# rohitsinghlab/SAME

Measured on AMD Instinct MI355X. Metric: cell-pairs/sec on 100k×100k cost build + edge-cross sweep; % HBM roofline, higher is better.
Workload: dtype f64

## Files before the change

### same_amd/csrc/common.h

```cpp
#pragma once
#include <hip/hip_runtime.h>

#include <cstdint>
#include <cstdio>
#include <cstring>
#include <string>
#include <vector>

#include "same_hip_diag.h"

struct ncclComm;

enum Slot {
    SL_A = 0, SL_R, SL_AXY, SL_RXY, SL_PAIRS, SL_OUT0, SL_OUT1, SL_OUT2, SL_TRIS, SL_MATCH,
    SL_SIGN, SL_SIZE, SL_TYPE, SL_FLAG0, SL_FLAG1, SL_FLAG2, SL_COUNTS, SL_X, SL_MASK,
    SL_K_HIST, SL_K_RANK, SL_K_SXY, SL_K_SIDX, SL_K_BBOX, SL_K_START,
    SL_Q_START, SL_Q_RANK, SL_Q_SXY, SL_Q_SIDX,
    SL_COUNT
};

struct same_spread_alloc {
    char *va = nullptr;
    size_t bytes = 0;
    std::vector<void *> handles;
// ... 102 lines not shown
}
template <typename T>
inline int up_as(same_ctx *ctx, Slot s, const T *host, size_t n, T **out) {
    void *p = nullptr;
    int rc = same_up(ctx, s, host, n * sizeof(T), &p);
    *out = static_cast<T *>(p);
    return rc;
}

static inline int64_t ceil_div(int64_t a, int64_t b) { return (a + b - 1) / b; }

int check_index_range(same_ctx *ctx, const int32_t *idx, int64_t n, int64_t lo, int64_t hi, const char *what);

struct same_pair_csr {
    std::vector<int32_t> prow, order, where, csr;
    std::vector<double> ccsr;
};
inline int same_pairs_by_row(same_ctx *ctx, const int32_t *pairs, const double *costs, int64_t P, int64_t n_m, int64_t n_r, same_pair_csr *out) {
    std::vector<int32_t> &prow = out->prow, &order = out->order, &where = out->where, &csr = out->csr;
    prow.assign((size_t)n_m + 1, 0);
    order.resize((size_t)P);
    where.resize((size_t)P);
    csr.resize((size_t)P * 2);
    out->ccsr.resize((size_t)P);
    for (int64_t p = 0; p < P; ++p) {
        const int32_t i = pairs[2 * p], j = pairs[2 * p + 1];
        REQUIRE(ctx, i >= 0 && i < n_m && j >= 0 && j < n_r);
        ++prow[(size_t)i + 1];
    }
    for (int64_t i = 0; i < n_m; ++i) prow[(size_t)i + 1] += prow[(size_t)i];
    {
        std::vector<int32_t> at(prow.begin(), prow.end() - 1);
        for (int64_t p = 0; p < P; ++p) {
            const int32_t q = at[(size_t)pairs[2 * p]]++;
            order[(size_t)q] = (int32_t)p;
            where[(size_t)p] = q;
        }
    }
    std::vector<int64_t> seen((size_t)n_r, -1);
    for (int64_t i = 0; i < n_m; ++i)
        for (int32_t q = prow[(size_t)i]; q < prow[(size_t)i + 1]; ++q) {
            const int32_t p = order[(size_t)q], j = pairs[2 * (int64_t)p + 1];
            if (seen[(size_t)j] == i) {
                ctx->err = "invalid argument: a (row, column) pair given twice";
                return SAME_EINVAL;
            }
            seen[(size_t)j] = i;
            csr[2 * (size_t)q] = (int32_t)i;
            csr[2 * (size_t)q + 1] = j;
            out->ccsr[(size_t)q] = costs[p];
        }
    return SAME_OK;
}

int same_pair_rowmin_core(same_ctx *ctx, const int32_t *dpairs, const double *dcosts, int64_t P, int64_t n_m, double *dout);
int same_greedy_core(same_ctx *ctx, const int32_t *dpairs, const double *dcosts, int64_t P, int64_t n_m, int64_t n_r,
                     const uint8_t *dprefer, int32_t *dmatch_pair, int *out_rounds);

constexpr int SAME_GREEDY_BATCH_MAX = 64;
struct same_greedy_state {
    uint8_t *alive = nullptr;
    uint8_t *used = nullptr;
    unsigned long long *key[2] = {nullptr, nullptr};
    unsigned *idx[2] = {nullptr, nullptr};
    unsigned long long *sel = nullptr;
    bool float_costs = false;
};
int same_greedy_rounds_core(same_ctx *ctx, const int32_t *dpairs, const double *dcosts, int64_t P, const unsigned long long *dP,
                            int64_t n_m, int64_t n_r, const same_greedy_state &st, int32_t *dmatch_pair, int first, int count);

constexpr int SAME_LAUNCH_WINDOWS = 8;
struct same_greedy_job {
    const int32_t *pairs = nullptr;
    const double *costs = nullptr;
    int64_t P = 0, n_m = 0, n_r = 0;
    same_greedy_state st;
    int32_t *match_pair = nullptr;
};
int same_greedy_rounds_batch_core(same_ctx *ctx, const same_greedy_job *jobs, int n_jobs, int first, int count);

int same_sort_u64_core(same_ctx *ctx, unsigned long long *dkey, int64_t n_pad);
int same_merge_dedup_core(same_ctx *ctx, const uint8_t *dviol, unsigned viol_mask, const int32_t *dwin, const int32_t *da, const int32_t *dr,
                          int64_t n, int32_t *dout, unsigned long long *dtotal);

struct same_knn_index;
struct same_knn_window_job {
    const int32_t *rows_m = nullptr;
    const unsigned long long *dn_m = nullptr;
    int64_t cap_m = 0;
    const int32_t *rows_r = nullptr;
    const unsigned long long *dn_r = nullptr;
    double box[4] = {0, 0, 0, 0};
    int32_t *idx = nullptr, *cnt = nullptr;
};
int same_knn_window_batch_core(same_ctx *ctx, const same_knn_index *ix, const double *dmov_xy, const same_knn_window_job *jobs, int n_jobs, int k);
struct same_cost_window_job {
    const int32_t *rows = nullptr;
    const unsigned long long *dn = nullptr;
    int64_t cap = 0;
    const int32_t *idx = nullptr;
    void *out = nullptr;
};
int same_padded_cost_window_batch_core(same_ctx *ctx, int cost_f32, const void *dA, const void *dR, int T, const void *daxy_c, const void *drxy_c,
                                       const same_cost_window_job *jobs, int n_jobs, int k, double w);
```

### same_amd/csrc/merge.hip

```cpp
#include <algorithm>

#include "common.h"
#include "scan.h"

namespace {

constexpr int SORT_BLOCK = 2048;

__global__ __launch_bounds__(256) void merge_key_kernel(const uint8_t *__restrict__ viol, unsigned viol_mask, const int32_t *__restrict__ window, int64_t n,
                                                          int64_t n_pad, unsigned long long *__restrict__ key) {
    const int64_t i = (int64_t)blockIdx.x * blockDim.x + threadIdx.x;
    if (i >= n_pad) return;
    key[i] = i < n ? ((unsigned long long)((viol[i] & viol_mask) ? 1 : 0) << 63) | ((unsigned long long)(uint32_t)window[i] << 32) | (unsigned long long)i
                   : ~0ull;
}

__global__ __launch_bounds__(256) void bitonic_global_kernel(unsigned long long *__restrict__ key, int64_t n_pad, int64_t j, int64_t k) {
    const int64_t t = (int64_t)blockIdx.x * blockDim.x + threadIdx.x;
    if (t >= n_pad / 2) return;
    const int64_t lo = ((t / j) * 2 * j) + (t % j), hi = lo + j;
    const bool up = (lo & k) == 0;
    const unsigned long long a = key[lo], b = key[hi];
    if ((a > b) == up) { key[lo] = b; key[hi] = a; }
}

__global__ __launch_bounds__(1024) void bitonic_lds_kernel(unsigned long long *__restrict__ key, int64_t k, int j_top) {
    __shared__ unsigned long long s[SORT_BLOCK];
    const int64_t base = (int64_t)blockIdx.x * SORT_BLOCK;
    s[threadIdx.x] = key[base + threadIdx.x];
    s[threadIdx.x + 1024] = key[base + threadIdx.x + 1024];
    __syncthreads();
    for (int j = j_top; j >= 1; j >>= 1) {
        const int t = threadIdx.x;
        const int lo = ((t / j) * 2 * j) + (t % j), hi = lo + j;
        const bool up = ((base + lo) & k) == 0;
        const unsigned long long a = s[lo], b = s[hi];
        if ((a > b) == up) { s[lo] = b; s[hi] = a; }
        __syncthreads();
    }
    key[base + threadIdx.x] = s[threadIdx.x];
    key[base + threadIdx.x + 1024] = s[threadIdx.x + 1024];
}

__global__ __launch_bounds__(1024) void bitonic_lds_head_kernel(unsigned long long *__restrict__ key) {
    __shared__ unsigned long long s[SORT_BLOCK];
    const int64_t base = (int64_t)blockIdx.x * SORT_BLOCK;
    s[threadIdx.x] = key[base + threadIdx.x];
    s[threadIdx.x + 1024] = key[base + threadIdx.x + 1024];
    __syncthreads();
    for (int k = 2; k <= SORT_BLOCK; k <<= 1)
        for (int j = k >> 1; j >= 1; j >>= 1) {
            const int t = threadIdx.x;
            const int lo = ((t / j) * 2 * j) + (t % j), hi = lo + j;
            const bool up = ((base + lo) & k) == 0;
            const unsigned long long a = s[lo], b = s[hi];
            if ((a > b) == up) { s[lo] = b; s[hi] = a; }
            __syncthreads();
        }
    key[base + threadIdx.x] = s[threadIdx.x];
    key[base + threadIdx.x + 1024] = s[threadIdx.x + 1024];
}

__device__ __forceinline__ uint64_t mix64(uint64_t x) {
    x ^= x >> 30; x *= 0xbf58476d1ce4e5b9ull;
    x ^= x >> 27; x *= 0x94d049bb133111ebull;
    return x ^ (x >> 31);
}

constexpr unsigned long long EMPTY = ~0ull;

__device__ __forceinline__ int64_t pair_slot(unsigned long long *__restrict__ tkey, int64_t mask, unsigned long long pair) {
    int64_t h = (int64_t)(mix64(pair) & (uint64_t)mask);
    for (;;) {
        const unsigned long long seen = atomicCAS(&tkey[h], EMPTY, pair);
        if (seen == EMPTY || seen == pair) return h;
        h = (h + 1) & mask;
    }
}

__global__ __launch_bounds__(256) void merge_first_kernel(const unsigned long long *__restrict__ key, int64_t n, const int32_t *__restrict__ a_code,
                                                            const int32_t *__restrict__ r_code, unsigned long long *__restrict__ tkey,
                                                            unsigned int *__restrict__ tfirst, int64_t mask) {
    const int64_t s = (int64_t)blockIdx.x * blockDim.x + threadIdx.x;
    if (s >= n) return;
    const uint32_t row = (uint32_t)key[s];
    const unsigned long long pair = ((unsigned long long)(uint32_t)a_code[row] << 32) | (uint32_t)r_code[row];
    atomicMin(&tfirst[pair_slot(tkey, mask, pair)], (unsigned int)s);
}

__global__ __launch_bounds__(scan::NT) void merge_compact_kernel(const unsigned long long *__restrict__ key, int64_t n, const int32_t *__restrict__ a_code,
                                                                  const int32_t *__restrict__ r_code, unsigned long long *__restrict__ tkey,
                                                                  const unsigned int *__restrict__ tfirst, int64_t mask,
                                                                  unsigned long long *__restrict__ status, int32_t *__restrict__ out_rows,
                                                                  unsigned long long *__restrict__ out_total) {
    __shared__ scan::Shared sh;
    auto keep_of = [&](int64_t q) -> bool {
        if (q >= n) return false;
        const uint32_t row = (uint32_t)key[q];
        const unsigned long long pair = ((unsigned long long)(uint32_t)a_code[row] << 32) | (uint32_t)r_code[row];
        return tfirst[pair_slot(tkey, mask, pair)] == (unsigned int)q;
    };
    const int64_t s0 = (int64_t)blockIdx.x * scan::NT + threadIdx.x;
    const bool keep = keep_of(s0);
    auto val = [&](int64_t q) { return scan::Pair{(q == s0 ? keep : keep_of(q)) ? 1u : 0u, 0u}; };
    scan::Pair through;
    const scan::Pair off = scan::exclusive(status, (int)blockIdx.x, val, sh, &through);
    if (keep) out_rows[off.a] = (int32_t)(uint32_t)key[s0];
    if (blockIdx.x == gridDim.x - 1 && threadIdx.x == 0) *out_total = through.a;
}

}

int same_sort_u64_core(same_ctx *ctx, unsigned long long *dkey, int64_t n_pad) {
    REQUIRE(ctx, n_pad >= SORT_BLOCK && (n_pad & (n_pad - 1)) == 0);
    hipLaunchKernelGGL(bitonic_lds_head_kernel, dim3((unsigned)(n_pad / SORT_BLOCK)), dim3(1024), 0, ctx->stream, dkey);
    for (int64_t k = 2 * SORT_BLOCK; k <= n_pad; k <<= 1) {
        for (int64_t j = k >> 1; j >= SORT_BLOCK; j >>= 1)
            hipLaunchKernelGGL(bitonic_global_kernel, dim3((unsigned)ceil_div(n_pad / 2, 256)), dim3(256), 0, ctx->stream, dkey, n_pad, j, k);
        hipLaunchKernelGGL(bitonic_lds_kernel, dim3((unsigned)(n_pad / SORT_BLOCK)), dim3(1024), 0, ctx->stream, dkey, k, SORT_BLOCK / 2);
    }
    HIP_TRY(ctx, hipGetLastError());
    return SAME_OK;
}

int same_merge_dedup_core(same_ctx *ctx, const uint8_t *dviol, unsigned viol_mask, const int32_t *dwin, const int32_t *da, const int32_t *dr,
                          int64_t n, int32_t *dout, unsigned long long *dtotal) {
    REQUIRE(ctx, n > 0 && n < ((int64_t)1 << 30));
    int64_t n_pad = SORT_BLOCK;
    while (n_pad < n) n_pad <<= 1;
    int64_t slots = 2;
    while (slots < 2 * n) slots <<= 1;
    unsigned long long *dkey, *dtkey, *dstatus;
    unsigned int *dtfirst;
    const size_t st_words = scan::status_bytes(n) / 8;
    SAME_TRY(slot_as(ctx, SL_X, (size_t)n_pad, &dkey));
    SAME_TRY(slot_as(ctx, SL_OUT0, (size_t)slots, &dtkey));
    SAME_TRY(slot_as(ctx, SL_OUT1, (size_t)slots, &dtfirst));
    SAME_TRY(slot_as(ctx, SL_MASK, st_words, &dstatus));
    SAME_FILL(ctx, dtkey, 0xFF, (size_t)slots * 8);
    SAME_FILL(ctx, dtfirst, 0xFF, (size_t)slots * 4);
    SAME_FILL(ctx, dstatus, 0, st_words * 8);
    SAME_LAUNCH(ctx, merge_key_kernel, dim3((unsigned)ceil_div(n_pad, 256)), dim3(256), 0, dviol, viol_mask, dwin, n, n_pad, dkey);
    SAME_TRY(same_sort_u64_core(ctx, dkey, n_pad));
    const unsigned grid = (unsigned)ceil_div(n, 256);
    SAME_LAUNCH(ctx, merge_first_kernel, dim3(grid), dim3(256), 0, dkey, n, da, dr, dtkey, dtfirst, slots - 1);
    SAME_LAUNCH(ctx, merge_compact_kernel, dim3(scan::blocks_for(n)), dim3(scan::NT), 0, dkey, n, da, dr, dtkey, dtfirst, slots - 1,
                scan::arg(dstatus), dout, dtotal);
    HIP_TRY(ctx, hipGetLastError());
    return SAME_OK;
}

extern "C" int same_merge_dedup(same_ctx *ctx, const uint8_t *viol, const int32_t *window_id, const int32_t *aligned_code,
                                const int32_t *ref_code, int64_t n, int32_t *out_rows, int64_t *out_n) {
    REQUIRE(ctx, ctx && out_n && n >= 0 && n < ((int64_t)1 << 30));
    *out_n = 0;
    if (n == 0) return SAME_OK;
    REQUIRE(ctx, viol && window_id && aligned_code && ref_code && out_rows);
    for (int64_t i = 0; i < n; ++i)
        if (window_id[i] < 0 || aligned_code[i] < 0 || ref_code[i] < 0) {
            ctx->err = "same_merge_dedup: window ids and id codes must be non-negative";
            return SAME_ERANGE;
        }
    SAME_TRY(same_use(ctx));
    uint8_t *dviol;
    int32_t *dwin, *da, *dr, *dout;
    unsigned long long *dtotal;
    SAME_TRY(up_as(ctx, SL_FLAG0, viol, (size_t)n, &dviol));
    SAME_TRY(up_as(ctx, SL_PAIRS, window_id, (size_t)n, &dwin));
    SAME_TRY(up_as(ctx, SL_MATCH, aligned_code, (size_t)n, &da));
    SAME_TRY(up_as(ctx, SL_TRIS, ref_code, (size_t)n, &dr));
    SAME_TRY(slot_as(ctx, SL_OUT2, (size_t)n + 4, &dout));
    dtotal = reinterpret_cast<unsigned long long *>(dout + (((size_t)n + 1) & ~size_t(1)));
    SAME_TRY(same_merge_dedup_core(ctx, dviol, 0xFFu, dwin, da, dr, n, dout, dtotal));
    unsigned long long total = 0;
    SAME_TRY(same_down(ctx, &total, dtotal, sizeof total));
    HIP_TRY(ctx, hipStreamSynchronize(ctx->stream));
    REQUIRE(ctx, (int64_t)total <= n);
    SAME_TRY(same_down(ctx, out_rows, dout, (size_t)total * sizeof(int32_t)));
    HIP_TRY(ctx, hipStreamSynchronize(ctx->stream));
    *out_n = (int64_t)total;
    return SAME_OK;
}
```

### same_amd/csrc/window_merge.hip

```cpp
#include "window_internal.h"


namespace {

using namespace devmath;
using namespace win;
using scan::Pair;

struct CollectArgs {
    const int32_t *match_row;
    const uint8_t *pflag;
    const int32_t *rows_ua;
    const double *axy;
    int64_t n;
    double tx0, tx1, ty0, ty1;
    int32_t wid, pos;
};

__device__ __forceinline__ bool central(const CollectArgs &w, int64_t c) {
    if (c >= w.n || w.match_row[c] < 0) return false;
    const double2_t p = ld2(w.axy, c);
    return p.x >= w.tx0 && p.x < w.tx1 && p.y >= w.ty0 && p.y < w.ty1;
}

// ... 23 lines not shown
                                                                  int64_t cap) {
    __shared__ scan::Shared sh;
    const CollectArgs &w = b.w[blockIdx.y];
    if ((int64_t)blockIdx.x * scan::NT >= w.n) return;
    auto val = [&](int64_t c) { return Pair{central(w, c) ? 1u : 0u, 0u}; };
    Pair through;
    const Pair off = scan::exclusive(status + blockIdx.y * status_stride, (int)blockIdx.x, val, sh, &through);
    const int64_t c = (int64_t)blockIdx.x * scan::NT + threadIdx.x;
    if (!central(w, c)) return;
    unsigned long long at = dcount[0] + off.a;
    for (unsigned q = 0; q < blockIdx.y; ++q) at += dcount[2 + q];
    if ((int64_t)at >= cap) return;
    acc.a_row[at] = w.rows_ua[c];
    acc.r_row[at] = w.match_row[c];
    acc.flags[at] = w.pflag[c];
    acc.wid[at] = w.wid;
    acc.pos[at] = w.pos;
    acc.cidx[at] = (int32_t)c;
}

__global__ void collect_bump_kernel(unsigned long long *dcount, int n_w) {
    unsigned long long add = 0;
    for (int q = 0; q < n_w; ++q) {
        add += dcount[2 + q];
        dcount[2 + q] = 0ull;
    }
    dcount[0] += add;
}

__global__ __launch_bounds__(256) void codes_kernel(const int32_t *__restrict__ a_row, const int32_t *__restrict__ r_row, int64_t n,
                                                     const int32_t *__restrict__ a_codes, const int32_t *__restrict__ r_codes,
                                                     int32_t *__restrict__ ac, int32_t *__restrict__ rc) {
    const int64_t i = (int64_t)blockIdx.x * blockDim.x + threadIdx.x;
    if (i >= n) return;
    ac[i] = a_codes ? a_codes[a_row[i]] : a_row[i];
    rc[i] = r_codes ? r_codes[r_row[i]] : r_row[i];
}

__global__ __launch_bounds__(256) void degree_kernel(const int32_t *__restrict__ kept, const unsigned long long *__restrict__ dm, int64_t bound,
                                                      const int32_t *__restrict__ ac, const int32_t *__restrict__ rc,
                                                      unsigned *__restrict__ deg_a, unsigned *__restrict__ deg_r) {
    const int64_t i = (int64_t)blockIdx.x * blockDim.x + threadIdx.x;
    if (i >= bound || i >= (int64_t)*dm) return;
    const int32_t row = kept[i];
    atomicAdd(&deg_a[ac[row]], 1u);
    atomicAdd(&deg_r[rc[row]], 1u);
}

struct SeamArgs {
    const int32_t *near_start;
    const double *near_boxes;
    const double *mov_xy, *ref_xy;
    int n_pos, all_seam;
    double reach;
};

__device__ __forceinline__ bool seam_of(const SeamArgs &s, int32_t pos, int32_t a_row, int32_t r_row) {
    if (s.all_seam) return true;
    if (!s.near_start) return false;
    if (pos < 0 || pos >= s.n_pos) return true;
    const int32_t b = s.near_start[pos], e = s.near_start[pos + 1];
    if (b == e) return false;
    const double2_t a = ld2(s.mov_xy, a_row), r = ld2(s.ref_xy, r_row);
    for (int32_t q = b; q < e; ++q) {
        const double x0 = s.near_boxes[4 * (int64_t)q], x1 = s.near_boxes[4 * (int64_t)q + 1], y0 = s.near_boxes[4 * (int64_t)q + 2],
                     y1 = s.near_boxes[4 * (int64_t)q + 3];
        if (a.x >= x0 && a.x < x1 && a.y >= y0 && a.y < y1) return true;
        if (r.x >= x0 - s.reach && r.x <= x1 + s.reach && r.y >= y0 - s.reach && r.y <= y1 + s.reach) return true;
    }
    return false;
}

__global__ __launch_bounds__(256) void classify_kernel(const int32_t *__restrict__ kept, const unsigned long long *__restrict__ dm, int64_t bound,
                                                        const int32_t *__restrict__ ac, const int32_t *__restrict__ rc,
                                                        const unsigned *__restrict__ deg_a, const unsigned *__restrict__ deg_r,
                                                        const int32_t *__restrict__ a_row, const int32_t *__restrict__ r_row,
                                                        const int32_t *__restrict__ pos, SeamArgs seams, uint8_t *__restrict__ cls,
                                                        int32_t *__restrict__ row_of) {
    const int64_t i = (int64_t)blockIdx.x * blockDim.x + threadIdx.x;
    if (i >= bound || i >= (int64_t)*dm) return;
    const int32_t row = kept[i];
    const bool lone = deg_a[ac[row]] == 1u && deg_r[rc[row]] == 1u;
    const bool seam = seam_of(seams, pos[row], a_row[row], r_row[row]);
    cls[i] = seam ? 3 : (lone ? 0 : 1);
    if (lone && !seam) row_of[ac[row]] = row;
}

__global__ __launch_bounds__(scan::NT) void rest_kernel(const int32_t *__restrict__ kept, const unsigned long long *__restrict__ dm,
                                                         const uint8_t *__restrict__ cls, const int32_t *__restrict__ ac,
                                                         const int32_t *__restrict__ rc, AccRows acc, unsigned long long *__restrict__ status,
                                                         RestRec *__restrict__ out, unsigned long long *__restrict__ out_total) {
    __shared__ scan::Shared sh;
    const int64_t m = (int64_t)*dm;
    auto val = [&](int64_t i) { return Pair{i < m && cls[i] != 0 ? 1u : 0u, 0u}; };
    Pair through;
    const Pair off = scan::exclusive(status, (int)blockIdx.x, val, sh, &through);
    const int64_t i = (int64_t)blockIdx.x * scan::NT + threadIdx.x;
    if (i < m && cls[i] != 0) {
        const int32_t row = kept[i];
        out[off.a] = RestRec{row, ac[row], rc[row], acc.wid[row], acc.pos[row], acc.cidx[row], (acc.flags[row] & 3u) | (cls[i] == 3 ? 4u : 0u)};
    }
    if (blockIdx.x == gridDim.x - 1 && threadIdx.x == 0) *out_total = through.a;
}

__global__ __launch_bounds__(256) void winners_kernel(const int32_t *__restrict__ rows, int64_t n, const int32_t *__restrict__ ac,
                                                       int32_t *__restrict__ row_of) {
    const int64_t i = (int64_t)blockIdx.x * blockDim.x + threadIdx.x;
    if (i < n) row_of[ac[rows[i]]] = rows[i];
}

__global__ __launch_bounds__(scan::NT) void final_kernel(const int32_t *__restrict__ row_of, int64_t n_codes, AccRows acc,
                                                          unsigned long long *__restrict__ status, FinalRec *__restrict__ out,
                                                          unsigned long long *__restrict__ out_total) {
    __shared__ scan::Shared sh;
    auto val = [&](int64_t c) { return Pair{c < n_codes && row_of[c] >= 0 ? 1u : 0u, 0u}; };
    Pair through;
    const Pair off = scan::exclusive(status, (int)blockIdx.x, val, sh, &through);
    const int64_t c = (int64_t)blockIdx.x * scan::NT + threadIdx.x;
    if (c < n_codes && row_of[c] >= 0) {
        const int32_t row = row_of[c];
        out[off.a] = FinalRec{acc.a_row[row], acc.r_row[row], acc.cidx[row], acc.wid[row], acc.pos[row], acc.flags[row] & 3u};
    }
    if (blockIdx.x == gridDim.x - 1 && threadIdx.x == 0) *out_total = through.a;
}

constexpr int MAX_EXTRA_COLUMNS = 4;
struct ExtraColumns {
    const unsigned long long *mov[MAX_EXTRA_COLUMNS], *ref[MAX_EXTRA_COLUMNS];
    int n_mov, n_ref;
};
__global__ __launch_bounds__(256) void table_columns_kernel(const FinalRec *__restrict__ rows, int64_t n, const double *__restrict__ mov_types, int T,
                                                            const double *__restrict__ mov_xy, const double *__restrict__ ref_xy, ExtraColumns ex,
                                                            unsigned long long *__restrict__ out) {
    const int64_t i = (int64_t)blockIdx.x * blockDim.x + threadIdx.x;
    if (i >= n) return;
    const FinalRec rec = rows[i];
    const int64_t a = rec.a_row, r = rec.r_row;
    const unsigned long long *__restrict__ t = reinterpret_cast<const unsigned long long *>(mov_types) + a * T;
    int64_t col = 0;
    for (int q = 0; q < T; ++q) out[(col++) * n + i] = t[q];
    const unsigned long long *pa = reinterpret_cast<const unsigned long long *>(mov_xy) + 2 * a,
                             *pr = reinterpret_cast<const unsigned long long *>(ref_xy) + 2 * r;
    out[(col++) * n + i] = pa[0];
    out[(col++) * n + i] = pa[1];
    out[(col++) * n + i] = pr[0];
    out[(col++) * n + i] = pr[1];
    for (int q = 0; q < ex.n_mov; ++q) out[(col++) * n + i] = ex.mov[q][a];
    for (int q = 0; q < ex.n_ref; ++q) out[(col++) * n + i] = ex.ref[q][r];
    out[(col++) * n + i] = (unsigned long long)(long long)rec.cidx;
    out[(col++) * n + i] = (unsigned long long)(long long)rec.wid;
    out[(col++) * n + i] = (unsigned long long)(long long)rec.pos;
    uint8_t *bytes = reinterpret_cast<uint8_t *>(out + col * n);
    bytes[i] = (uint8_t)((rec.flags >> 1) & 1u);
    bytes[n + i] = (uint8_t)(rec.flags & 1u);
}

AccRows rows_of(const same_merge_acc *a) { return AccRows{a->a_row, a->r_row, a->wid, a->pos, a->cidx, a->flags}; }

void free_rows(same_merge_acc *a) {
    for (void *p : {(void *)a->a_row, (void *)a->r_row, (void *)a->wid, (void *)a->pos, (void *)a->cidx, (void *)a->flags})
        if (p) (void)hipFree(p);
    a->a_row = a->r_row = a->wid = a->pos = a->cidx = nullptr;
    a->flags = nullptr;
    a->cap = 0;
}

int reserve_rows(same_merge_acc *a, int64_t need, int64_t have) {
    if (need <= a->cap) return SAME_OK;
    same_ctx *ctx = a->ctx;
    HIP_TRY(ctx, hipStreamSynchronize(ctx->stream));
    const int64_t cap = std::max<int64_t>(need + need / 4, 4096);
    int32_t **fields[5] = {&a->a_row, &a->r_row, &a->wid, &a->pos, &a->cidx};
    int32_t *olds[5], *news[5] = {nullptr, nullptr, nullptr, nullptr, nullptr};
    uint8_t *old_flags = a->flags, *new_flags = nullptr;
    for (int q = 0; q < 5; ++q) olds[q] = *fields[q];
    hipError_t e = hipSuccess;
    for (int q = 0; q < 5 && e == hipSuccess; ++q) {
        e = hipMalloc(reinterpret_cast<void **>(&news[q]), (size_t)cap * sizeof(int32_t));
        if (e == hipSuccess && have) e = hipMemcpyAsync(news[q], olds[q], (size_t)have * sizeof(int32_t), hipMemcpyDeviceToDevice, ctx->stream);
    }
    if (e == hipSuccess) e = hipMalloc(reinterpret_cast<void **>(&new_flags), (size_t)cap);
    if (e == hipSuccess && have) e = hipMemcpyAsync(new_flags, old_flags, (size_t)have, hipMemcpyDeviceToDevice, ctx->stream);
    if (e == hipSuccess) e = hipStreamSynchronize(ctx->stream);
    if (e != hipSuccess) {
        for (int q = 0; q < 5; ++q)
// ... 145 lines not shown
    a->loaded_codes_a = n_codes_a;
    a->loaded_codes_r = n_codes_r;
    const unsigned long long cnt[2] = {(unsigned long long)n, 0ull};
    SAME_COPY(ctx, a->dcount, cnt, sizeof cnt, hipMemcpyHostToDevice);
    if (n) {
        int32_t *const dst[5] = {a->a_row, a->r_row, a->wid, a->pos, a->cidx};
        const int32_t *const src[5] = {a_code, r_code, window_ids, pos, cidx};
        for (int f = 0; f < 5; ++f) SAME_COPY(ctx, dst[f], src[f], (size_t)n * sizeof(int32_t), hipMemcpyHostToDevice);
        SAME_COPY(ctx, a->flags, flags, (size_t)n, hipMemcpyHostToDevice);
    }
    SAME_WAIT(ctx);
    return SAME_OK;
}

int same_window_collect(same_window *const *windows, int n_windows, same_merge_acc *a, const double *trims, const int32_t *window_ids,
                        const int32_t *plan_pos) {
    same_ctx *ctx = nullptr;
    SAME_TRY(check_batch(windows, n_windows, &ctx));
    REQUIRE(ctx, a && a->ctx == ctx && trims && window_ids && plan_pos && !a->resolved);
    int64_t add = 0;
    for (int i = 0; i < n_windows; ++i) {
        REQUIRE(ctx, windows[i]->has_results() && window_ids[i] >= 0);
        add += windows[i]->cur.n_ua;
    }
    REQUIRE(ctx, a->bound + add < ((int64_t)1 << 30));
    SAME_TRY(same_use(ctx));
    if (a->bound + add > a->cap) {
        unsigned long long have = 0;
        HIP_TRY(ctx, hipMemcpyAsync(&have, a->dcount, sizeof have, hipMemcpyDeviceToHost, ctx->stream));
        HIP_TRY(ctx, hipStreamSynchronize(ctx->stream));
        SAME_TRY(reserve_rows(a, a->bound + add, (int64_t)have));
    }
    a->bound += add;
    int64_t most = 0;
    for (int i = 0; i < n_windows; ++i) most = std::max(most, windows[i]->cur.n_ua);
    const int64_t stride = (int64_t)(scan::status_bytes(most) / 8);
    SAME_TRY(ensure(ctx, a->scan_words, (size_t)stride * 8 * SAME_LAUNCH_WINDOWS));
    unsigned long long *words = static_cast<unsigned long long *>(a->scan_words.p);
    for (int g = 0; g < n_windows; g += SAME_LAUNCH_WINDOWS) {
        Batch<CollectArgs> b{};
        int n_g = 0;
        int64_t most_g = 0;
        for (int i = g; i < n_windows && i < g + SAME_LAUNCH_WINDOWS; ++i) {
            const same_window *w = windows[i];
            if (w->cur.n_ua == 0) continue;
            const double *t = trims + 4 * i;
            b.w[n_g++] = CollectArgs{w->match_row, w->pflag, w->cur.rows_ua, w->cur.axy_c, w->cur.n_ua, t[0], t[1], t[2], t[3], window_ids[i], plan_pos[i]};
            most_g = std::max(most_g, w->cur.n_ua);
        }
        if (!n_g) continue;
        const dim3 grid(scan::blocks_for(most_g), (unsigned)n_g);
        SAME_LAUNCH(ctx, collect_count_kernel, grid, dim3(scan::NT), 0, b, a->dcount + 2, words, stride);
        SAME_LAUNCH(ctx, collect_write_kernel, grid, dim3(scan::NT), 0, b, a->dcount, scan::arg(words), stride, rows_of(a), a->cap);
        SAME_LAUNCH(ctx, collect_bump_kernel, dim3(1), dim3(1), 0, a->dcount, n_g);
    }
    HIP_TRY(ctx, hipGetLastError());
    return SAME_OK;
}

int same_merge_acc_resolve(same_merge_acc *const *accs, int n_accs, const same_section *mov, const same_section *ref, int64_t *out_counts) {
    if (!accs || n_accs < 1 || !accs[0]) return SAME_EINVAL;
    same_merge_acc *a = accs[0];
    same_ctx *ctx = a->ctx;
    REQUIRE(ctx, n_accs <= 64 && out_counts);
    const bool loaded = a->loaded != 0;
    REQUIRE(ctx, loaded ? n_accs == 1 : (mov && ref && mov->ctx->device == ctx->device && ref->ctx->device == ctx->device));
    for (int q = 0; q < n_accs; ++q) {
        REQUIRE(ctx, accs[q] && accs[q]->ctx->device == ctx->device && !accs[q]->resolved);
        for (int p = 0; p < q; ++p) REQUIRE(ctx, accs[p] != accs[q]);
    }
    for (int q = 0; q < 4; ++q) out_counts[q] = 0;
    SAME_TRY(same_use(ctx));
    int64_t n = 0;
    SAME_TRY(lay_end_to_end(accs, n_accs, &n));
    for (int q = 0; q < n_accs; ++q) accs[q]->resolved = 1;
    a->n_rows = n;
    a->n_codes_a = loaded ? a->loaded_codes_a : (mov->id_codes ? mov->n_codes : mov->n);
    const int64_t n_codes_a = std::max<int64_t>(a->n_codes_a, 1),
                  n_codes_r = std::max<int64_t>(loaded ? a->loaded_codes_r : (ref->id_codes ? ref->n_codes : ref->n), 1);
    const int32_t *codes_a = loaded ? nullptr : mov->id_codes, *codes_r = loaded ? nullptr : ref->id_codes;
    const int64_t nn = std::max<int64_t>(n, 1);
    unsigned long long *status, *counters;
    unsigned *deg_a, *deg_r;
    int32_t *kept;
    uint8_t *cls;
    size_t zero_bytes = 0;
    auto lay = [&](Carver cv) {
        status = cv.scan_words(nn);
        counters = cv.take<unsigned long long>(8);
        deg_a = cv.take<unsigned>((size_t)n_codes_a);
        deg_r = cv.take<unsigned>((size_t)n_codes_r);
        zero_bytes = cv.off;
        a->row_of = cv.take<int32_t>((size_t)n_codes_a);
        a->ac = cv.take<int32_t>((size_t)nn);
        a->rc = cv.take<int32_t>((size_t)nn);
        kept = cv.take<int32_t>((size_t)nn);
        cls = cv.take<uint8_t>((size_t)nn);
        return cv.off;
    };
    SAME_TRY(ensure(ctx, a->work, lay(Carver())));
    lay(Carver(a->work.p));
    SAME_FILL(ctx, a->work.p, 0, zero_bytes);
    SAME_FILL(ctx, a->row_of, 0xFF, (size_t)n_codes_a * 4);
    a->counters = counters;
    SAME_TRY(ensure(ctx, a->out, (size_t)nn * sizeof(RestRec)));
    RestRec *rest = static_cast<RestRec *>(a->out.p);
    if (n) {
        SAME_LAUNCH(ctx, codes_kernel, dim3(grid_for(n)), dim3(256), 0, a->a_row, a->r_row, n, codes_a, codes_r, a->ac, a->rc);
        SAME_TRY(same_merge_dedup_core(ctx, a->flags, 1u, a->wid, a->ac, a->rc, n, kept, counters));
        SAME_LAUNCH(ctx, degree_kernel, dim3(grid_for(n)), dim3(256), 0, kept, counters, n, a->ac, a->rc, deg_a, deg_r);
        const SeamArgs seams{a->n_pos ? static_cast<const int32_t *>(a->near_start.p) : nullptr, static_cast<const double *>(a->near_boxes.p),
                             loaded ? nullptr : mov->xy, loaded ? nullptr : ref->xy, a->n_pos, a->all_seam, a->reach};
        SAME_LAUNCH(ctx, classify_kernel, dim3(grid_for(n)), dim3(256), 0, kept, counters, n, a->ac, a->rc, deg_a, deg_r, a->a_row, a->r_row, a->pos,
                    seams, cls, a->row_of);
        SAME_LAUNCH(ctx, rest_kernel, dim3(scan::blocks_for(n)), dim3(scan::NT), 0, kept, counters, cls, a->ac, a->rc, rows_of(a), scan::arg(status), rest,
                    counters + 1);
        HIP_TRY(ctx, hipGetLastError());
        unsigned long long hc[2] = {0, 0};
        SAME_COPY(ctx, hc, counters, sizeof hc, hipMemcpyDeviceToHost);
        SAME_WAIT(ctx);
        REQUIRE(ctx, (int64_t)hc[0] <= n && (int64_t)hc[1] <= (int64_t)hc[0]);
        a->n_kept = (int64_t)hc[0];
        a->n_rest = (int64_t)hc[1];
    }
    a->host.resize((size_t)a->n_rest * sizeof(RestRec) + 64);
    if (a->n_rest) {
        SAME_COPY(ctx, a->host.data(), rest, (size_t)a->n_rest * sizeof(RestRec), hipMemcpyDeviceToHost);
        SAME_WAIT(ctx);
    }
    out_counts[0] = a->n_rows;
    out_counts[1] = a->n_kept;
    out_counts[2] = a->n_rest;
    out_counts[3] = a->n_kept - a->n_rest;
    return SAME_OK;
}

int same_merge_acc_plain(same_merge_acc *const *accs, int n_accs, int64_t *out_n_rows) {
    if (!accs || n_accs < 1 || !accs[0]) return SAME_EINVAL;
    same_merge_acc *a = accs[0];
    same_ctx *ctx = a->ctx;
    REQUIRE(ctx, n_accs <= 64 && out_n_rows && !a->loaded);
    for (int q = 0; q < n_accs; ++q) {
        REQUIRE(ctx, accs[q] && accs[q]->ctx->device == ctx->device && !accs[q]->resolved);
        for (int p = 0; p < q; ++p) REQUIRE(ctx, accs[p] != accs[q]);
    }
    *out_n_rows = 0;
    SAME_TRY(same_use(ctx));
    int64_t n = 0;
    SAME_TRY(lay_end_to_end(accs, n_accs, &n));
    for (int q = 0; q < n_accs; ++q) accs[q]->resolved = 2;
    a->n_rows = a->n_kept = a->n_final = n;
    a->n_rest = 0;
    a->final_on_host = 0;
    a->merged = 0;
    SAME_TRY(ensure(ctx, a->out, (size_t)std::max<int64_t>(n, 1) * sizeof(FinalRec)));
    if (n) SAME_LAUNCH(ctx, plain_kernel, dim3(grid_for(n)), dim3(256), 0, rows_of(a), n, static_cast<FinalRec *>(a->out.p));
    HIP_TRY(ctx, hipGetLastError());
    *out_n_rows = n;
    return SAME_OK;
}

int same_merge_acc_finish(same_merge_acc *a, const int32_t *winner_rows, int64_t n_winners, int64_t *out_n_final) {
    if (!a) return SAME_EINVAL;
    same_ctx *ctx = a->ctx;
    REQUIRE(ctx, a->resolved && a->row_of && out_n_final && n_winners >= 0 && n_winners <= a->n_rest && (n_winners == 0 || winner_rows));
    *out_n_final = 0;
    SAME_TRY(same_use(ctx));
    SAME_TRY(check_index_range(ctx, winner_rows, n_winners, 0, std::max<int64_t>(a->n_rows, 1), "winner rows"));
    const int64_t n_codes = std::max<int64_t>(a->n_codes_a, 1);
    unsigned long long *counters = a->counters, *status2 = nullptr;
    SAME_TRY(slot_as(ctx, SL_MASK, scan::status_bytes(n_codes) / 8, &status2));
    SAME_FILL(ctx, status2, 0, scan::status_bytes(n_codes));
    if (n_winners) {
        int32_t *dw = nullptr;
        SAME_TRY(up_as(ctx, SL_MATCH, winner_rows, (size_t)n_winners, &dw));
        SAME_LAUNCH(ctx, winners_kernel, dim3(grid_for(n_winners)), dim3(256), 0, dw, n_winners, a->ac, a->row_of);
    }
    SAME_TRY(ensure(ctx, a->out, (size_t)std::max<int64_t>(a->n_kept, 1) * sizeof(FinalRec)));
    FinalRec *fin = static_cast<FinalRec *>(a->out.p);
    SAME_LAUNCH(ctx, final_kernel, dim3(scan::blocks_for(n_codes)), dim3(scan::NT), 0, a->row_of, a->n_codes_a, rows_of(a), scan::arg(status2), fin,
                counters + 2);
    HIP_TRY(ctx, hipGetLastError());
    unsigned long long total = 0;
    SAME_COPY(ctx, &total, counters + 2, sizeof total, hipMemcpyDeviceToHost);
    SAME_WAIT(ctx);
    REQUIRE(ctx, (int64_t)total <= a->n_kept);
    a->n_final = (int64_t)total;
    a->final_on_host = 0;
    a->merged = 1;
    a->resolved = 2;
    *out_n_final = a->n_final;
    return SAME_OK;
}

int same_merge_acc_columns(same_merge_acc *a, const same_section *mov, const same_section *ref, const void *const *extra_mov, int n_extra_mov,
                           const void *const *extra_ref, int n_extra_ref, void *out_host, int64_t n_final) {
    return same_merge_acc_columns_layer(a, mov, nullptr, ref, extra_mov, n_extra_mov, extra_ref, n_extra_ref, out_host, n_final);
}

int same_merge_acc_columns_layer(same_merge_acc *a, const same_section *mov, const same_types_layer *layer, const same_section *ref,
                                 const void *const *extra_mov, int n_extra_mov, const void *const *extra_ref, int n_extra_ref, void *out_host,
                                 int64_t n_final) {
    if (!a) return SAME_EINVAL;
    same_ctx *ctx = a->ctx;
    REQUIRE(ctx, !layer || (mov && layer->sec == mov && layer->ctx->device == ctx->device));
    const double *types64 = !mov ? nullptr : layer ? layer->types64 : mov->types64;
    REQUIRE(ctx, a->resolved == 2 && !a->loaded && mov && ref && n_final == a->n_final && (n_final == 0 || out_host));
    REQUIRE(ctx, mov->ctx->device == ctx->device && ref->ctx->device == ctx->device && (mov->T == 0 || types64));
    REQUIRE(ctx, n_extra_mov >= 0 && n_extra_mov <= MAX_EXTRA_COLUMNS && n_extra_ref >= 0 && n_extra_ref <= MAX_EXTRA_COLUMNS);
// ... 70 lines not shown
```

Baseline: 620.1 billion.

## Replace full-sort merge dedup with hash-table min-key winners and sort only rest rows

The merge dedup no longer bitonic-sorts every row to find the first occurrence of each (a,r) pair. Instead, a hash table keyed by pair keeps the minimum sort key through atomicMin, and a scan compacts the winners in row order. Only the much smaller set of rest rows is then sorted by key to keep the output order deterministic, and their records are built after the sort. This removes an O(n log^2 n) sort over all rows, at the cost of an extra sort over the rest subset and a change of cls indexing from kept position to row.

```diff
diff --git a/same_amd/csrc/common.h b/same_amd/csrc/common.h
--- a/same_amd/csrc/common.h
+++ b/same_amd/csrc/common.h
@@ -208,6 +208,10 @@
 int same_sort_u64_core(same_ctx *ctx, unsigned long long *dkey, int64_t n_pad);
 int same_merge_dedup_core(same_ctx *ctx, const uint8_t *dviol, unsigned viol_mask, const int32_t *dwin, const int32_t *da, const int32_t *dr,
                           int64_t n, int32_t *dout, unsigned long long *dtotal);
+int same_merge_winners_core(same_ctx *ctx, const uint8_t *dviol, unsigned viol_mask, const int32_t *dwin, const int32_t *da, const int32_t *dr,
+                            int64_t n, int32_t *dout, unsigned long long *dtotal);
+int same_merge_sorted_keys_core(same_ctx *ctx, const uint8_t *dviol, unsigned viol_mask, const int32_t *dwin, const int32_t *drows, int64_t m,
+                                const unsigned long long **dsorted);
 
 struct same_knn_index;
 struct same_knn_window_job {
diff --git a/same_amd/csrc/merge.hip b/same_amd/csrc/merge.hip
--- a/same_amd/csrc/merge.hip
+++ b/same_amd/csrc/merge.hip
@@ -6,13 +6,24 @@
 namespace {
 
 constexpr int SORT_BLOCK = 2048;
+
+__device__ __forceinline__ unsigned long long key_of(const uint8_t *__restrict__ viol, unsigned viol_mask, const int32_t *__restrict__ window, int64_t i) {
+    return ((unsigned long long)((viol[i] & viol_mask) ? 1 : 0) << 63) | ((unsigned long long)(uint32_t)window[i] << 32) | (unsigned long long)i;
+}
 
 __global__ __launch_bounds__(256) void merge_key_kernel(const uint8_t *__restrict__ viol, unsigned viol_mask, const int32_t *__restrict__ window, int64_t n,
                                                           int64_t n_pad, unsigned long long *__restrict__ key) {
     const int64_t i = (int64_t)blockIdx.x * blockDim.x + threadIdx.x;
     if (i >= n_pad) return;
-    key[i] = i < n ? ((unsigned long long)((viol[i] & viol_mask) ? 1 : 0) << 63) | ((unsigned long long)(uint32_t)window[i] << 32) | (unsigned long long)i
-                   : ~0ull;
+    key[i] = i < n ? key_of(viol, viol_mask, window, i) : ~0ull;
+}
+
+__global__ __launch_bounds__(256) void merge_listed_key_kernel(const uint8_t *__restrict__ viol, unsigned viol_mask, const int32_t *__restrict__ window,
+                                                                 const int32_t *__restrict__ rows, int64_t m, int64_t n_pad,
+                                                                 unsigned long long *__restrict__ key) {
+    const int64_t i = (int64_t)blockIdx.x * blockDim.x + threadIdx.x;
+    if (i >= n_pad) return;
+    key[i] = i < m ? key_of(viol, viol_mask, window, rows[i]) : ~0ull;
 }
 
 __global__ __launch_bounds__(256) void bitonic_global_kernel(unsigned long long *__restrict__ key, int64_t n_pad, int64_t j, int64_t k) {
@@ -69,10 +80,11 @@
 
 constexpr unsigned long long EMPTY = ~0ull;
 
+template <int STRIDE = 1>
 __device__ __forceinline__ int64_t pair_slot(unsigned long long *__restrict__ tkey, int64_t mask, unsigned long long pair) {
     int64_t h = (int64_t)(mix64(pair) & (uint64_t)mask);
     for (;;) {
-        const unsigned long long seen = atomicCAS(&tkey[h], EMPTY, pair);
+        const unsigned long long seen = atomicCAS(&tkey[STRIDE * h], EMPTY, pair);
         if (seen == EMPTY || seen == pair) return h;
         h = (h + 1) & mask;
     }
@@ -106,6 +118,35 @@
     scan::Pair through;
     const scan::Pair off = scan::exclusive(status, (int)blockIdx.x, val, sh, &through);
     if (keep) out_rows[off.a] = (int32_t)(uint32_t)key[s0];
+    if (blockIdx.x == gridDim.x - 1 && threadIdx.x == 0) *out_total = through.a;
+}
+
+__global__ __launch_bounds__(256) void merge_best_kernel(const uint8_t *__restrict__ viol, unsigned viol_mask, const int32_t *__restrict__ window, int64_t n,
+                                                           const int32_t *__restrict__ a_code, const int32_t *__restrict__ r_code,
+                                                           unsigned long long *__restrict__ tab, int64_t mask, uint32_t *__restrict__ slot_of) {
+    const int64_t i = (int64_t)blockIdx.x * blockDim.x + threadIdx.x;
+    if (i >= n) return;
+    const unsigned long long pair = ((unsigned long long)(uint32_t)a_code[i] << 32) | (uint32_t)r_code[i];
+    const int64_t h = pair_slot<2>(tab, mask, pair);
+    atomicMin(&tab[2 * h + 1], key_of(viol, viol_mask, window, i));
+    slot_of[i] = (uint32_t)h;
+}
+
+__global__ __launch_bounds__(scan::NT) void merge_winners_kernel(const uint8_t *__restrict__ viol, unsigned viol_mask, const int32_t *__restrict__ window,
+                                                                  int64_t n, const unsigned long long *__restrict__ tab,
+                                                                  const uint32_t *__restrict__ slot_of, unsigned long long *__restrict__ status,
+                                                                  int32_t *__restrict__ out_rows, unsigned long long *__restrict__ out_total) {
+    __shared__ scan::Shared sh;
+    auto keep_of = [&](int64_t q) -> bool {
+        if (q >= n) return false;
+        return tab[2 * (int64_t)slot_of[q] + 1] == key_of(viol, viol_mask, window, q);
+    };
+    const int64_t i0 = (int64_t)blockIdx.x * scan::NT + threadIdx.x;
+    const bool keep = keep_of(i0);
+    auto val = [&](int64_t q) { return scan::Pair{(q == i0 ? keep : keep_of(q)) ? 1u : 0u, 0u}; };
+    scan::Pair through;
+    const scan::Pair off = scan::exclusive(status, (int)blockIdx.x, val, sh, &through);
+    if (keep) out_rows[off.a] = (int32_t)i0;
     if (blockIdx.x == gridDim.x - 1 && threadIdx.x == 0) *out_total = through.a;
 }
 
@@ -147,6 +188,39 @@
     SAME_LAUNCH(ctx, merge_compact_kernel, dim3(scan::blocks_for(n)), dim3(scan::NT), 0, dkey, n, da, dr, dtkey, dtfirst, slots - 1,
                 scan::arg(dstatus), dout, dtotal);
     HIP_TRY(ctx, hipGetLastError());
+    return SAME_OK;
+}
+
+int same_merge_winners_core(same_ctx *ctx, const uint8_t *dviol, unsigned viol_mask, const int32_t *dwin, const int32_t *da, const int32_t *dr,
+                            int64_t n, int32_t *dout, unsigned long long *dtotal) {
+    REQUIRE(ctx, n > 0 && n < ((int64_t)1 << 30));
+    int64_t slots = 2;
+    while (slots < 2 * n) slots <<= 1;
+    unsigned long long *dtab, *dstatus;
+    const size_t st_words = scan::status_bytes(n) / 8;
+    uint32_t *dslot_of;
+    SAME_TRY(slot_as(ctx, SL_OUT0, (size_t)slots * 2, &dtab));
+    SAME_TRY(slot_as(ctx, SL_OUT1, (size_t)n, &dslot_of));
+    SAME_TRY(slot_as(ctx, SL_MASK, st_words, &dstatus));
+    SAME_FILL(ctx, dtab, 0xFF, (size_t)slots * 16);
+    SAME_FILL(ctx, dstatus, 0, st_words * 8);
+    SAME_LAUNCH(ctx, merge_best_kernel, dim3((unsigned)ceil_div(n, 256)), dim3(256), 0, dviol, viol_mask, dwin, n, da, dr, dtab, slots - 1, dslot_of);
+    SAME_LAUNCH(ctx, merge_winners_kernel, dim3(scan::blocks_for(n)), dim3(scan::NT), 0, dviol, viol_mask, dwin, n, dtab, dslot_of, scan::arg(dstatus),
+                dout, dtotal);
+    HIP_TRY(ctx, hipGetLastError());
+    return SAME_OK;
+}
+
+int same_merge_sorted_keys_core(same_ctx *ctx, const uint8_t *dviol, unsigned viol_mask, const int32_t *dwin, const int32_t *drows, int64_t m,
+                                const unsigned long long **dsorted) {
+    REQUIRE(ctx, m > 0 && m < ((int64_t)1 << 30) && dsorted);
+    int64_t n_pad = SORT_BLOCK;
+    while (n_pad < m) n_pad <<= 1;
+    unsigned long long *dkey;
+    SAME_TRY(slot_as(ctx, SL_X, (size_t)n_pad, &dkey));
+    SAME_LAUNCH(ctx, merge_listed_key_kernel, dim3((unsigned)ceil_div(n_pad, 256)), dim3(256), 0, dviol, viol_mask, dwin, drows, m, n_pad, dkey);
+    SAME_TRY(same_sort_u64_core(ctx, dkey, n_pad));
+    *dsorted = dkey;
     return SAME_OK;
 }
 
diff --git a/same_amd/csrc/window_merge.hip b/same_amd/csrc/window_merge.hip
--- a/same_amd/csrc/window_merge.hip
+++ b/same_amd/csrc/window_merge.hip
@@ -129,25 +129,31 @@
     const int32_t row = kept[i];
     const bool lone = deg_a[ac[row]] == 1u && deg_r[rc[row]] == 1u;
     const bool seam = seam_of(seams, pos[row], a_row[row], r_row[row]);
-    cls[i] = seam ? 3 : (lone ? 0 : 1);
+    cls[row] = seam ? 3 : (lone ? 0 : 1);
     if (lone && !seam) row_of[ac[row]] = row;
 }
 
-__global__ __launch_bounds__(scan::NT) void rest_kernel(const int32_t *__restrict__ kept, const unsigned long long *__restrict__ dm,
-                                                         const uint8_t *__restrict__ cls, const int32_t *__restrict__ ac,
-                                                         const int32_t *__restrict__ rc, AccRows acc, unsigned long long *__restrict__ status,
-                                                         RestRec *__restrict__ out, unsigned long long *__restrict__ out_total) {
+__global__ __launch_bounds__(scan::NT) void rest_rows_kernel(const int32_t *__restrict__ kept, const unsigned long long *__restrict__ dm,
+                                                              const uint8_t *__restrict__ cls, unsigned long long *__restrict__ status,
+                                                              int32_t *__restrict__ out_rows, unsigned long long *__restrict__ out_total) {
     __shared__ scan::Shared sh;
     const int64_t m = (int64_t)*dm;
-    auto val = [&](int64_t i) { return Pair{i < m && cls[i] != 0 ? 1u : 0u, 0u}; };
+    auto val = [&](int64_t i) { return Pair{i < m && cls[kept[i]] != 0 ? 1u : 0u, 0u}; };
     Pair through;
     const Pair off = scan::exclusive(status, (int)blockIdx.x, val, sh, &through);
     const int64_t i = (int64_t)blockIdx.x * scan::NT + threadIdx.x;
-    if (i < m && cls[i] != 0) {
-        const int32_t row = kept[i];
-        out[off.a] = RestRec{row, ac[row], rc[row], acc.wid[row], acc.pos[row], acc.cidx[row], (acc.flags[row] & 3u) | (cls[i] == 3 ? 4u : 0u)};
-    }
+    if (i < m && cls[kept[i]] != 0) out_rows[off.a] = kept[i];
     if (blockIdx.x == gridDim.x - 1 && threadIdx.x == 0) *out_total = through.a;
+}
+
+__global__ __launch_bounds__(256) void rest_records_kernel(const unsigned long long *__restrict__ sorted, int64_t m, int64_t n,
+                                                            const uint8_t *__restrict__ cls, const int32_t *__restrict__ ac,
+                                                            const int32_t *__restrict__ rc, AccRows acc, RestRec *__restrict__ out) {
+    const int64_t i = (int64_t)blockIdx.x * blockDim.x + threadIdx.x;
+    if (i >= m) return;
+    const int32_t row = (int32_t)(uint32_t)sorted[i];
+    if ((int64_t)(uint32_t)row >= n) return;
+    out[i] = RestRec{row, ac[row], rc[row], acc.wid[row], acc.pos[row], acc.cidx[row], (acc.flags[row] & 3u) | (cls[row] == 3 ? 4u : 0u)};
 }
 
 __global__ __launch_bounds__(256) void winners_kernel(const int32_t *__restrict__ rows, int64_t n, const int32_t *__restrict__ ac,
@@ -459,7 +465,7 @@
     const int64_t nn = std::max<int64_t>(n, 1);
     unsigned long long *status, *counters;
     unsigned *deg_a, *deg_r;
-    int32_t *kept;
+    int32_t *kept, *rest_rows;
     uint8_t *cls;
     size_t zero_bytes = 0;
     auto lay = [&](Carver cv) {
@@ -472,6 +478,7 @@
         a->ac = cv.take<int32_t>((size_t)nn);
         a->rc = cv.take<int32_t>((size_t)nn);
         kept = cv.take<int32_t>((size_t)nn);
+        rest_rows = cv.take<int32_t>((size_t)nn);
         cls = cv.take<uint8_t>((size_t)nn);
         return cv.off;
     };
@@ -484,14 +491,13 @@
     RestRec *rest = static_cast<RestRec *>(a->out.p);
     if (n) {
         SAME_LAUNCH(ctx, codes_kernel, dim3(grid_for(n)), dim3(256), 0, a->a_row, a->r_row, n, codes_a, codes_r, a->ac, a->rc);
-        SAME_TRY(same_merge_dedup_core(ctx, a->flags, 1u, a->wid, a->ac, a->rc, n, kept, counters));
+        SAME_TRY(same_merge_winners_core(ctx, a->flags, 1u, a->wid, a->ac, a->rc, n, kept, counters));
         SAME_LAUNCH(ctx, degree_kernel, dim3(grid_for(n)), dim3(256), 0, kept, counters, n, a->ac, a->rc, deg_a, deg_r);
         const SeamArgs seams{a->n_pos ? static_cast<const int32_t *>(a->near_start.p) : nullptr, static_cast<const double *>(a->near_boxes.p),
                              loaded ? nullptr : mov->xy, loaded ? nullptr : ref->xy, a->n_pos, a->all_seam, a->reach};
         SAME_LAUNCH(ctx, classify_kernel, dim3(grid_for(n)), dim3(256), 0, kept, counters, n, a->ac, a->rc, deg_a, deg_r, a->a_row, a->r_row, a->pos,
                     seams, cls, a->row_of);
-        SAME_LAUNCH(ctx, rest_kernel, dim3(scan::blocks_for(n)), dim3(scan::NT), 0, kept, counters, cls, a->ac, a->rc, rows_of(a), scan::arg(status), rest,
-                    counters + 1);
+        SAME_LAUNCH(ctx, rest_rows_kernel, dim3(scan::blocks_for(n)), dim3(scan::NT), 0, kept, counters, cls, scan::arg(status), rest_rows, counters + 1);
         HIP_TRY(ctx, hipGetLastError());
         unsigned long long hc[2] = {0, 0};
         SAME_COPY(ctx, hc, counters, sizeof hc, hipMemcpyDeviceToHost);
@@ -502,6 +508,10 @@
     }
     a->host.resize((size_t)a->n_rest * sizeof(RestRec) + 64);
     if (a->n_rest) {
+        const unsigned long long *sorted = nullptr;
+        SAME_TRY(same_merge_sorted_keys_core(ctx, a->flags, 1u, a->wid, rest_rows, a->n_rest, &sorted));
+        SAME_LAUNCH(ctx, rest_records_kernel, dim3(grid_for(a->n_rest)), dim3(256), 0, sorted, a->n_rest, n, cls, a->ac, a->rc, rows_of(a), rest);
+        HIP_TRY(ctx, hipGetLastError());
         SAME_COPY(ctx, a->host.data(), rest, (size_t)a->n_rest * sizeof(RestRec), hipMemcpyDeviceToHost);
         SAME_WAIT(ctx);
     }
```

Result: no change. 620.1 billion (-0.0%).
